# ebiggers/libdeflate

Hardware: AMD Instinct MI355X
Metric: compress+decompress MB/s, 64 KiB chunks level 6 (higher is better)
Workload: dtype u8

## Files before the change

### libdeflate_amd/csrc/checksum_kernels.hip

```cpp
#include "device_common.h"
#include "kernels.h"

#define CRC_POLY 0xEDB88320u
#define ROW 1024u

static __device__ __forceinline__ u32 gf2_mulmod(u32 a, u32 b)
{
	u32 p = 0;
#pragma unroll 8
	for (int i = 31; i >= 0; i--) {
		p ^= b & (0u - ((a >> i) & 1u));
		b = (b >> 1) ^ (CRC_POLY & (0u - (b & 1u)));
	}
	return p;
}

struct crc_lds {
	u32 stride[16][256];
	u32 t0[256];
};

static __device__ __forceinline__ u32
crc_row_generic(const crc_lds &L, const u32 *__restrict__ xpow8,
		const u8 *__restrict__ p, u32 len, u32 reg, u32 lane)
{
	u32 start = lane * 16;
	u32 r = (lane == 0) ? reg : 0;
	u32 part = 0;

	if (start < len) {
		u32 m = len - start;
		if (m > 16)
			m = 16;
		for (u32 k = 0; k < m; k++)
			r = L.t0[(r ^ p[start + k]) & 0xFF] ^ (r >> 8);
		part = gf2_mulmod(xpow8[len - start - m], r);
	} else if (lane == 0) {
		part = r;
	}
	return wave_xor(part);
}

static __device__ __forceinline__ u32
crc_row_full_final(const crc_lds &L, const u32 *__restrict__ xpow8,
		   uint4 v, u32 reg_lane, u32 lane)
{
	u32 w[4] = { v.x ^ reg_lane, v.y, v.z, v.w };
	u32 r = 0;
#pragma unroll
	for (int i = 0; i < 4; i++) {
#pragma unroll
		for (int j = 0; j < 4; j++)
			r = L.t0[(r ^ (w[i] >> (8 * j))) & 0xFF] ^ (r >> 8);
	}
	return wave_xor(gf2_mulmod(xpow8[(63 - lane) * 16], r));
}

extern "C" __global__ void __launch_bounds__(256)
lda_crc32_batch_kernel(u64 n_chunks, const u8 *__restrict__ base,
		       const u64 *__restrict__ offsets,
		       const u64 *__restrict__ nbytes,
		       const u32 *__restrict__ init,
		       u32 *__restrict__ out,
		       const u32 *__restrict__ g_tables ,
		       const u32 *__restrict__ xpow8 )
{
	__shared__ crc_lds L;
	const u32 lane = threadIdx.x & 63;
	const u32 wave = threadIdx.x >> 6;

	for (u32 i = threadIdx.x; i < 17 * 256; i += 256)
		((u32 *)&L)[i] = g_tables[i];
	__syncthreads();

	for (u64 c = (u64)blockIdx.x * 4 + wave; c < n_chunks;
	     c += (u64)gridDim.x * 4) {
		const u8 *p = base + offsets[c];
		u64 n = nbytes[c];
		u32 reg = ~(init ? init[c] : 0u);

		u32 head = (u32)((0 - (uintptr_t)p) & 15);
		if (head > n)
			head = (u32)n;
		if (head) {
			reg = crc_row_generic(L, xpow8, p, head, reg, lane);
			p += head;
			n -= head;
		}
		u64 rows = n / ROW;
		if (rows) {
			const uint4 *q = (const uint4 *)p + lane;
			u32 r = (lane == 0) ? reg : 0;
			uint4 v = q[0];
			for (u64 row = 0; row + 1 < rows; row++) {
				uint4 nv = q[(row + 1) * 64];
				u32 w0 = v.x ^ r, w1 = v.y, w2 = v.z, w3 = v.w;
				r = L.stride[0][w0 & 0xFF] ^
				    L.stride[1][(w0 >> 8) & 0xFF] ^
				    L.stride[2][(w0 >> 16) & 0xFF] ^
				    L.stride[3][w0 >> 24] ^
				    L.stride[4][w1 & 0xFF] ^
				    L.stride[5][(w1 >> 8) & 0xFF] ^
				    L.stride[6][(w1 >> 16) & 0xFF] ^
				    L.stride[7][w1 >> 24] ^
				    L.stride[8][w2 & 0xFF] ^
				    L.stride[9][(w2 >> 8) & 0xFF] ^
				    L.stride[10][(w2 >> 16) & 0xFF] ^
				    L.stride[11][w2 >> 24] ^
				    L.stride[12][w3 & 0xFF] ^
				    L.stride[13][(w3 >> 8) & 0xFF] ^
				    L.stride[14][(w3 >> 16) & 0xFF] ^
				    L.stride[15][w3 >> 24];
				v = nv;
			}
			reg = crc_row_full_final(L, xpow8, v, r, lane);
			p += rows * ROW;
			n -= rows * ROW;
		}
		if (n)
			reg = crc_row_generic(L, xpow8, p, (u32)n, reg, lane);
		if (lane == 0)
			out[c] = ~reg;
	}
}


#define ADLER_MOD 65521u
#define ADLER_SEG (1u << 24)

static __device__ __forceinline__ u32 dot4(u32 bytes, u32 weights, u32 acc)
{
	return __builtin_amdgcn_udot4(bytes, weights, acc, false);
}

extern "C" __global__ void __launch_bounds__(256)
lda_adler32_batch_kernel(u64 n_chunks, const u8 *__restrict__ base,
			 const u64 *__restrict__ offsets,
			 const u64 *__restrict__ nbytes,
			 const u32 *__restrict__ init,
			 u32 *__restrict__ out)
{
	const u32 lane = threadIdx.x & 63;
	const u32 wave = threadIdx.x >> 6;

	for (u64 c = (u64)blockIdx.x * 4 + wave; c < n_chunks;
	     c += (u64)gridDim.x * 4) {
		const u8 *p = base + offsets[c];
		u64 left = nbytes[c];
		u32 a0 = init ? init[c] : 1u;
		u64 s1 = a0 & 0xFFFF, s2 = a0 >> 16;

		while (left) {
			u32 n = left > ADLER_SEG ? ADLER_SEG : (u32)left;
			u64 S = 0, W = 0;
			u32 pos = 0;
			u32 head = (u32)((0 - (uintptr_t)p) & 15);

			if (head > n)
				head = n;
			if (lane < head) {
				u32 b = p[lane];
				S += b;
				W += (u64)(n - lane) * b;
			}
			pos = head;
			u32 rows = (n - pos) / ROW;
			const uint4 *q = (const uint4 *)(p + pos) + lane;
			for (u32 row = 0; row < rows; row++) {
				uint4 v = q[(u64)row * 64];
				u32 o = pos + row * ROW + lane * 16;
				u32 bs = dot4(v.x, 0x01010101u, 0);
				bs = dot4(v.y, 0x01010101u, bs);
				bs = dot4(v.z, 0x01010101u, bs);
				bs = dot4(v.w, 0x01010101u, bs);
				u32 ks = dot4(v.x, 0x03020100u, 0);
				ks = dot4(v.y, 0x07060504u, ks);
				ks = dot4(v.z, 0x0B0A0908u, ks);
				ks = dot4(v.w, 0x0F0E0D0Cu, ks);
				S += bs;
				W += (u64)(n - o) * bs - ks;
			}
			pos += rows * ROW;
			for (u32 i = pos + lane; i < n; i += 64) {
				u32 b = p[i];
				S += b;
				W += (u64)(n - i) * b;
			}
			S = wave_sum64(S);
			W = wave_sum64(W);
			s2 = (s2 + (u64)n % ADLER_MOD * s1 + W % ADLER_MOD) % ADLER_MOD;
			s1 = (s1 + S) % ADLER_MOD;
			p += n;
			left -= n;
		}
		if (lane == 0)
			out[c] = (u32)((s2 << 16) | s1);
	}
}

extern "C" __global__ void
lda_dict_prep_kernel(const u8 *__restrict__ dict, u64 dict_nbytes, u32 tail,
		     u32 pre_len, u32 sinfo, u8 *__restrict__ blk)
{
	if (threadIdx.x == 0) {
		((u32 *)blk)[0] = sinfo;
		((u64 *)blk)[2] = 0;
		((u64 *)blk)[3] = dict_nbytes;
	}
	const u32 skip = pre_len - tail;
	const u8 *src = dict + dict_nbytes - tail;
	for (u32 i = threadIdx.x; i < pre_len; i += blockDim.x)
		blk[64 + i] = i < skip ? 0 : src[i - skip];
}
```

### libdeflate_amd/csrc/host_common.h

```cpp
#ifndef LDA_HOST_COMMON_H
#define LDA_HOST_COMMON_H

#include <hip/hip_runtime.h>
#include <stddef.h>
#include <stdint.h>
#include <atomic>
#include <exception>
#include <functional>
#include <mutex>

#include "../../include/libdeflate_amd.h"

namespace lda {

void set_error(const char *fmt, ...);

#define LDA_HIP_TRY(expr, failret)                                           \
	do {                                                                 \
		hipError_t e_ = (expr);                                      \
		if (e_ != hipSuccess) {                                      \
			lda::set_error("%s: %s", #expr, hipGetErrorString(e_)); \
			return failret;                                      \
		}                                                            \
	} while (0)
// ... 5 lines not shown
	} while (0)
#define LDA_TRY(expr) LDA_HIP_TRY(expr, false)

struct DeviceCtx {
	int device = -1;
	int num_cus = 0;
	uint32_t *d_crc_tables = nullptr;
	uint32_t *d_crc_xpow8 = nullptr;
	std::mutex stage_mu;
	void *d_stage = nullptr;
	size_t stage_cap = 0;
	std::atomic<bool> deflate_attr_set{false}, inflate_attr_set{false}, stream_attr_set{false};
	std::atomic<int> sizes_waves_fit{0};
};

DeviceCtx *device_ctx();
bool device_selfcheck(int num_cus, uint64_t out[5]);

struct DeviceGuard {
	int prev = -1;
	bool switched = false, good = true;
	explicit DeviceGuard(int device);
	~DeviceGuard();
	bool ok() const { return good; }
	DeviceGuard(const DeviceGuard &) = delete;
	DeviceGuard &operator=(const DeviceGuard &) = delete;
};

struct EnvCfg {
	bool no_small = false;
	bool no_segments = false;
	int inflate_lpw = 0;
	bool inflate_par = true;
	int inflate_waves_per_cu = 16;
	int sizes_waves_per_cu = 0;
	int host_threads = 4;
	size_t seg_bytes = 0;
	bool no_stream_par = false;
	size_t stream_par_min = 16384;
	size_t zip_large_min = (size_t)128 << 10;
	size_t stream_window = 0;
	size_t stream_chunk = 0;
	int devices = 1;
	bool no_selfcheck = false;
	bool bgzf_serial = false;
	bool tar_serial = false;
	bool fanout_oversub = false;
	bool compress_overlap = true;
	int compress_tail_rounds = 0;
};
const EnvCfg &env_cfg();

void *stage_reserve(DeviceCtx *ctx, size_t nbytes);

[[noreturn]] void die(const char *what);

void complain(const char *what, int status);

struct PinnedPair {
	uint8_t *buf[2] = { nullptr, nullptr };
	hipEvent_t ev[2] = { nullptr, nullptr };
	size_t cap = 0;
	bool ensure(size_t want);
	void release();
};
struct PinnedBuf {
// ... 92 lines not shown
```

### libdeflate_amd/csrc/host_context.hip

```cpp
#include <stdarg.h>
#include <stdio.h>
#include <stdlib.h>
#include <string.h>
#include <pthread.h>
#include <algorithm>
#include <condition_variable>
#include <deque>
#include <functional>
#include <memory>
#include <thread>
#include <vector>

#include "host_common.h"
#include "kernels.h"

namespace lda {

static thread_local char g_err[512] = "";

void set_error(const char *fmt, ...)
{
	va_list ap;
	va_start(ap, fmt);
	vsnprintf(g_err, sizeof(g_err), fmt, ap);
	va_end(ap);
}

[[noreturn]] void die(const char *what)
{
	fprintf(stderr,
		"libdeflate_amd: %s failed on the gfx950 device (%s) and this "
		"call has no error return. This library has no CPU fallback.\n",
		what, g_err);
	abort();
}

void complain(const char *what, int status)
{
	fprintf(stderr, "libdeflate_amd: %s: status %d (%s)\n", what, status, g_err);
}

static EnvCfg read_env()
{
	EnvCfg c;
	c.no_small = getenv("LDA_NO_SMALL") != nullptr;
	c.no_segments = getenv("LDA_NO_SEGMENTS") != nullptr;
	if (const char *e = getenv("LDA_INFLATE_LPW")) {
		int v = atoi(e);
		if (v >= 1 && v <= 64)
			c.inflate_lpw = v;
	}
	if (const char *e = getenv("LDA_INFLATE_PAR"))
		c.inflate_par = atoi(e) != 0;
	if (const char *e = getenv("LDA_HOST_THREADS")) {
		int v = atoi(e);
		if (v >= 1 && v <= 16)
			c.host_threads = v;
	}
	if (const char *e = getenv("LDA_INFLATE_WAVES_PER_CU")) {
		int v = atoi(e);
		if (v >= 1 && v <= 16)
			c.inflate_waves_per_cu = v;
	}
	if (const char *e = getenv("LDA_SIZES_WAVES_PER_CU")) {
		int v = atoi(e);
		if (v >= 1 && v <= 32)
			c.sizes_waves_per_cu = v;
	}
	if (const char *e = getenv("LDA_SEG_BYTES")) {
		size_t v = (size_t)strtoull(e, nullptr, 0);
		if (v >= 8192 && v <= 65536 && v % 4096 == 0)
			c.seg_bytes = v;
	}
	c.no_stream_par = getenv("LDA_NO_STREAM_PAR") != nullptr;
	if (const char *e = getenv("LDA_STREAM_PAR_MIN"))
		c.stream_par_min = (size_t)strtoull(e, nullptr, 0);
	if (const char *e = getenv("LDA_ZIP_LARGE_MIN")) {
		size_t v = (size_t)strtoull(e, nullptr, 0);
		if (v >= 1)
			c.zip_large_min = v;
	}
	if (const char *e = getenv("LDA_STREAM_WINDOW")) {
		c.stream_window = (size_t)strtoull(e, nullptr, 0);
		if (c.stream_window && c.stream_window < 32768)
			c.stream_window = 32768;
	}
// ... 554 lines not shown

int span_out(PinnedPair *pp, const uint8_t *d_base, uint64_t d_off, uint8_t *dst, size_t n,
	     hipStream_t st, size_t piece)
{
	const size_t P = piece ? piece : span_piece(n), np = (n + P - 1) / P;
	std::vector<void *> outs(np);
	std::vector<uint64_t> nb(np), off(np);
	for (size_t i = 0; i < np; i++) {
		outs[i] = dst + i * P;
		nb[i] = i + 1 < np ? P : n - i * P;
		off[i] = d_off + i * P;
	}
	return copy_out_packed(pp, d_base, np, outs.data(), nb.data(), off.data(), st);
}

#define MAX_DEVICES 16
static DeviceCtx g_ctx[MAX_DEVICES];
static std::mutex g_ctx_mu;

static void gen_crc_tables(uint32_t *tab , uint32_t *xpow )
{
	const uint32_t poly = 0xEDB88320u;
	uint32_t t0[256];

	for (uint32_t b = 0; b < 256; b++) {
		uint32_t r = b;
		for (int k = 0; k < 8; k++)
			r = (r >> 1) ^ (poly & (0u - (r & 1u)));
		t0[b] = r;
	}
	for (uint32_t b = 0; b < 256; b++) {
		uint32_t r = t0[b];
		int zeros = 0;
		for (int k = 15; k >= 0; k--) {
			int want = (15 - k) + 1008;
			for (; zeros < want; zeros++)
				r = t0[r & 0xFF] ^ (r >> 8);
			tab[k * 256 + b] = r;
		}
	}
	memcpy(tab + 16 * 256, t0, sizeof(t0));
	uint32_t x = 0x80000000u;
	for (int d = 0; d < 1024; d++) {
		xpow[d] = x;
		for (int k = 0; k < 8; k++)
			x = (x >> 1) ^ (poly & (0u - (x & 1u)));
	}
}

bool device_selfcheck(int num_cus, uint64_t out[5])
{
	const unsigned blocks = (unsigned)(num_cus > 0 ? num_cus : 256);
	const unsigned waves = 16 * blocks;
	const size_t region = lda_selfcheck_region_bytes();
	uint8_t *buf = nullptr;
	uint64_t *d_cnt = nullptr;

	memset(out, 0, 5 * sizeof(uint64_t));
	LDA_HIP_TRY(hipMalloc((void **)&buf, (size_t)waves * region + 64), false);
	d_cnt = (uint64_t *)(buf + (size_t)waves * region);
	hipError_t e = hipMemset(buf, 0, (size_t)waves * region + 64);
	if (e == hipSuccess) {
		hipLaunchKernelGGL(lda_selfcheck_lds_order_kernel, dim3(blocks), dim3(1024), 0, 0,
				   d_cnt);
		hipLaunchKernelGGL(lda_selfcheck_visibility_kernel, dim3(waves), dim3(64), 0, 0,
				   buf, d_cnt);
		e = hipGetLastError();
	}
	if (e == hipSuccess)
		e = hipMemcpy(out, d_cnt, 5 * sizeof(uint64_t), hipMemcpyDeviceToHost);
	(void)hipFree(buf);
	if (e != hipSuccess) {
		set_error("hardware self-check: %s", hipGetErrorString(e));
		return false;
// ... 22 lines not shown
		good = false;
		return;
	}
	switched = true;
}

DeviceGuard::~DeviceGuard()
{
	if (switched && prev >= 0)
		(void)hipSetDevice(prev);
}

DeviceCtx *device_ctx()
{
	int dev = -1;
	hipError_t e = hipGetDevice(&dev);

	if (e != hipSuccess || dev < 0 || dev >= MAX_DEVICES) {
		set_error("hipGetDevice: %s", hipGetErrorString(e));
		return nullptr;
	}
	std::lock_guard<std::mutex> lk(g_ctx_mu);
	DeviceCtx *c = &g_ctx[dev];
	if (c->device == dev)
		return c;

	hipDeviceProp_t prop;
	LDA_HIP_TRY(hipGetDeviceProperties(&prop, dev), nullptr);
	if (strncmp(prop.gcnArchName, "gfx950", 6) != 0) {
		set_error("device %d is %s, this build targets gfx950 only",
			  dev, prop.gcnArchName);
		return nullptr;
	}
	static uint32_t tab[LDA_CRC_TABLE_WORDS], xpow[LDA_CRC_XPOW_WORDS];
	gen_crc_tables(tab, xpow);
	uint32_t *d_tab = nullptr;
	LDA_HIP_TRY(hipMalloc((void **)&d_tab, sizeof(tab) + sizeof(xpow)), nullptr);
	hipError_t ce = hipMemcpy(d_tab, tab, sizeof(tab), hipMemcpyHostToDevice);
	if (ce == hipSuccess)
		ce = hipMemcpy(d_tab + LDA_CRC_TABLE_WORDS, xpow, sizeof(xpow),
			       hipMemcpyHostToDevice);
	if (ce != hipSuccess) {
		(void)hipFree(d_tab);
		set_error("hipMemcpy(CRC tables): %s", hipGetErrorString(ce));
		return nullptr;
	}
	if (!env_cfg().no_selfcheck) {
		uint64_t sc[5];
		if (!device_selfcheck(prop.multiProcessorCount, sc)) {
			(void)hipFree(d_tab);
			return nullptr;
		}
	}
	c->d_crc_tables = d_tab;
	c->d_crc_xpow8 = d_tab + LDA_CRC_TABLE_WORDS;
	c->num_cus = prop.multiProcessorCount;
	c->device = dev;
	return c;
}

void *stage_reserve(DeviceCtx *ctx, size_t nbytes)
{
	if (nbytes <= ctx->stage_cap)
		return ctx->d_stage;
	size_t cap = align_up(nbytes + nbytes / 4 + 4096, 4096);
	void *p = nullptr;
	if (ctx->d_stage)
		(void)hipFree(ctx->d_stage);
	ctx->d_stage = nullptr;
	ctx->stage_cap = 0;
	hipError_t e = hipMalloc(&p, cap);
	if (e != hipSuccess) {
		set_error("hipMalloc(%zu): %s", cap, hipGetErrorString(e));
		return nullptr;
// ... 34 lines not shown
```

### libdeflate_amd/csrc/host_decompress.hip

```cpp
#include <stdio.h>
#include <stdlib.h>
#include <atomic>
#include <new>
#include <string.h>
#include <vector>

#include "host_objects.h"
#include "kernels.h"

namespace lda {

malloc_func_t g_malloc = nullptr;
free_func_t g_free = nullptr;

void *DevBuf::reserve(size_t n)
{
	if (n <= cap)
		return p;
	release();
	size_t want = align_up(n + n / 8 + 4096, 4096);
	hipError_t e = hipMalloc(&p, want);
	if (e != hipSuccess) {
		p = nullptr;
		set_error("hipMalloc(%zu): %s", want, hipGetErrorString(e));
// ... 171 lines not shown
	if (dict) {
		dlen = (uint32_t)(dict_nbytes < 32768 ? dict_nbytes : 32768);
		dtail = (const uint8_t *)d_dict + dict_nbytes - dlen;
		uint8_t *blk = s + blk_at;
		hipLaunchKernelGGL(lda_dict_prep_kernel, dim3(1), dim3(64), 0, st,
				   (const uint8_t *)d_dict, (uint64_t)dict_nbytes, 0u, 0u, 0u, blk);
		LDA_HIP_TRY(hipGetLastError(), LIBDEFLATE_AMD_NO_DEVICE);
		if (format == LIBDEFLATE_AMD_ZLIB) {
			dict_id = (uint32_t *)(blk + 4);
			int rc = libdeflate_amd_adler32_batch(1, d_dict, (const uint64_t *)(blk + 16),
							      (const uint64_t *)(blk + 24), NULL, dict_id,
							      stream);
			if (rc != LIBDEFLATE_AMD_OK)
				return rc;
		}
	}
	uint32_t *sums = (uint32_t *)s;
	uint64_t *ain = d_actual_in ? d_actual_in : (uint64_t *)(s + sums_bytes);
	uint64_t *aout = d_actual_out ? d_actual_out :
			 (uint64_t *)(s + sums_bytes + 8 * n);
	int exact_fill = d_actual_out == NULL;

	uint32_t lpw_max = 64;
	while (lda_inflate_lds_per_stream() * lpw_max + lda_inflate_lds_shared() > 163840)
		lpw_max >>= 1;
	uint32_t lpw = 2;
	while (lpw < lpw_max && (size_t)lpw * 32 * (size_t)c->num_cus < n)
		lpw <<= 1;
	if (env_cfg().inflate_lpw)
		lpw = (uint32_t)env_cfg().inflate_lpw;
	if (lpw > lpw_max)
		lpw = lpw_max;
	const bool par = env_cfg().inflate_par;
	if (!c->inflate_attr_set.load(std::memory_order_acquire)) {
		LDA_HIP_TRY(hipFuncSetAttribute(
				(const void *)lda_inflate_batch_kernel,
				hipFuncAttributeMaxDynamicSharedMemorySize,
				(int)(lda_inflate_lds_per_stream() * lpw_max +
				      lda_inflate_lds_shared())),
			    LIBDEFLATE_AMD_NO_DEVICE);
		c->inflate_attr_set.store(true, std::memory_order_release);
	}
	if (par) {
		const size_t grid_max = (size_t)c->num_cus * inflate_waves_per_cu();
		size_t grid = grid_max < n ? grid_max : n;
		const size_t tok_bytes = grid * lda_inflate_tokcap() * 4;
		uint32_t *tok = (uint32_t *)d->tokens.reserve(inflate_tokens_bytes(n, c->num_cus));
		if (!tok)
			return LIBDEFLATE_AMD_OOM;
		uint32_t *next = (uint32_t *)((uint8_t *)tok + tok_bytes);
		LDA_HIP_TRY(hipMemsetAsync(next, 0, 16, st), LIBDEFLATE_AMD_NO_DEVICE);
		uint32_t *order = NULL;
		if (n > grid && n < 0xFFFFFFFFull) {
			order = (uint32_t *)(s + sums_bytes + 16 * n);
			hipLaunchKernelGGL(lda_inflate_order_kernel, dim3(1), dim3(1024), 0, st,
					   (uint64_t)n, d_in_nbytes, d_out_avail, order);
		}
		size_t lds = inflate_wave_lds();
		hipLaunchKernelGGL(lda_inflate_wave_kernel, dim3((unsigned)grid),
				   dim3(64), lds, st, (uint64_t)n, format, tok, next,
				   (const uint32_t *)order,
				   (const uint8_t *)d_in, d_in_offsets, d_in_nbytes,
				   (uint8_t *)d_out, d_out_offsets, d_out_avail,
				   d_results, ain, aout, dtail, dlen, (const uint32_t *)dict_id);
	} else {
		size_t lds = lda_inflate_lds_per_stream() * lpw +
			     lda_inflate_lds_shared();
		hipLaunchKernelGGL(lda_inflate_batch_kernel,
				   dim3((unsigned)((n + lpw - 1) / lpw)), dim3(64),
				   lds, st, (uint64_t)n, format, lpw,
				   (const uint8_t *)d_in, d_in_offsets, d_in_nbytes,
				   (uint8_t *)d_out, d_out_offsets, d_out_avail,
				   d_results, ain, aout, dtail, dlen, (const uint32_t *)dict_id);
	}
	LDA_HIP_TRY(hipGetLastError(), LIBDEFLATE_AMD_NO_DEVICE);
	if (format != LIBDEFLATE_AMD_DEFLATE) {
		int rc = format == LIBDEFLATE_AMD_GZIP ?
			libdeflate_amd_crc32_batch(n, d_out, d_out_offsets, aout,
						   NULL, sums, stream) :
			libdeflate_amd_adler32_batch(n, d_out, d_out_offsets,
						     aout, NULL, sums, stream);
		if (rc != LIBDEFLATE_AMD_OK)
			return rc;
	}
	if (format != LIBDEFLATE_AMD_DEFLATE || exact_fill) {
		hipLaunchKernelGGL(lda_inflate_finalize_kernel,
				   dim3((unsigned)((n + 255) / 256)), dim3(256), 0,
				   st, (uint64_t)n, format, exact_fill,
				   (const uint8_t *)d_in, d_in_offsets, d_out_avail,
				   sums, d_results, ain, aout);
		LDA_HIP_TRY(hipGetLastError(), LIBDEFLATE_AMD_NO_DEVICE);
	}
	return LIBDEFLATE_AMD_OK;
}

extern "C" LIBDEFLATEAPI int
libdeflate_amd_decompress_batch(struct libdeflate_decompressor *d, int format,
				size_t n, const void *d_in,
				const uint64_t *d_in_offsets,
				const uint64_t *d_in_nbytes, void *d_out,
				const uint64_t *d_out_offsets,
				const uint64_t *d_out_avail, int32_t *d_results,
				uint64_t *d_actual_in, uint64_t *d_actual_out,
				void *stream)
{
	return decompress_batch_impl(d, format, n, d_in, d_in_offsets, d_in_nbytes, d_out,
				     d_out_offsets, d_out_avail, d_results, d_actual_in,
				     d_actual_out, stream);
// ... 420 lines not shown
```

### libdeflate_amd/csrc/inflate_kernel.hip

```cpp
#include "device_common.h"
#include "kernels.h"

#ifndef PAR_PRIO
#define PAR_PRIO 1
#endif
#ifndef LIT_TB
#define LIT_TB 10
#endif
#ifndef LIT_TB_MIN
#define LIT_TB_MIN 9
#endif
#ifndef OFF_TB
#define OFF_TB 8
#endif
#ifndef OFF_TB_MIN
#define OFF_TB_MIN 7
#endif
#define TB_BIG_BLOCK 8192u

#define K_LIT (0u << 14)
#define K_LEN (1u << 14)
#define K_EOB (2u << 14)
#define ENTRY(kind, payload, len) ((u16)((kind) | ((payload) << 4) | (len)))

// ... 2100 lines not shown
			u64 ain = (CONSUMED() + 7) / 8;
			if (ain > in_n)
				result = LDA_BAD_DATA;
			else if (!COUNT || actual_in)
				actual_in[c] = hdr + ain;
		}
		if (COUNT) {
			if (result == LDA_SUCCESS && format == LDA_FMT_GZIP) {
				const u8 *p = inp + (CONSUMED() + 7) / 8;
				const u32 isize = p[4] | ((u32)p[5] << 8) | ((u32)p[6] << 16) |
						  ((u32)p[7] << 24);
				if (isize != (u32)out_pos)
					result = LDA_BAD_DATA;
			}
			if (result == LDA_SUCCESS && actual_in && format != LDA_FMT_DEFLATE)
				actual_in[c] += format == LDA_FMT_GZIP ? 8 : 4;
			if (result != LDA_SUCCESS && actual_in)
				actual_in[c] = 0;
			results[c] = result;
			actual_out[c] = result == LDA_SUCCESS ? out_pos : 0;
			return;
		}
		results[c] = result;
		actual_out[c] = result == LDA_SUCCESS ? out_pos :
				PREFIX && result == LDA_PREFIX ? out_avail : 0;
		if (result != LDA_SUCCESS)
			actual_in[c] = 0;
	}
}
#undef ltb
#undef otb

#ifndef LDA_INFLATE_DEVICE_ONLY
extern "C" __global__ void __launch_bounds__(64, 4)
lda_inflate_batch_kernel(u64 n_chunks, int format, u32 lpw,
			 const u8 *__restrict__ in_base,
			 const u64 *__restrict__ in_offsets,
			 const u64 *__restrict__ in_nbytes,
			 u8 *__restrict__ out_base,
			 const u64 *__restrict__ out_offsets,
			 const u64 *__restrict__ out_avail_arr,
			 s32 *__restrict__ results,
			 u64 *__restrict__ actual_in,
			 u64 *__restrict__ actual_out,
			 const u8 *__restrict__ dict, u32 dict_len,
			 const u32 *__restrict__ dict_id)
{
	lu8 *lds_raw = (lu8 *)(uintptr_t)0;

	inflate_block(blockIdx.x, lds_raw, 0, NULL, n_chunks, format, lpw, in_base,
		      in_offsets, in_nbytes, out_base, out_offsets, out_avail_arr,
		      results, actual_in, actual_out, dict, dict_len, dict_id);
}

#ifndef PAR_WAVES_PER_SIMD
#define PAR_WAVES_PER_SIMD 4
#endif
static __device__ __forceinline__ u32
order_bucket(const u64 *__restrict__ in_nbytes, const u64 *__restrict__ out_avail, u64 i)
{
	u64 b = in_nbytes[i];
	if (out_avail && b + (b >> 5) >= out_avail[i])
		b >>= 4;
	b >>= 9;
	return 255 - (b < 255 ? (u32)b : 255u);
}

extern "C" __global__ void __launch_bounds__(1024)
lda_inflate_order_kernel(u64 n, const u64 *__restrict__ in_nbytes,
			 const u64 *__restrict__ out_avail,
			 u32 *__restrict__ order)
{
	__shared__ u32 cnt[256], at[256];
	const u32 tid = threadIdx.x;

	if (tid < 256)
		cnt[tid] = 0;
	__syncthreads();
	for (u64 i = tid; i < n; i += 1024)
		atomicAdd(&cnt[order_bucket(in_nbytes, out_avail, i)], 1u);
	__syncthreads();
	if (tid < 64) {
		u32 v[4], s = 0;
#pragma unroll
		for (u32 k = 0; k < 4; k++) {
			v[k] = cnt[4 * tid + k];
			s += v[k];
		}
		u32 base = wave_scan_incl(s) - s;
#pragma unroll
		for (u32 k = 0; k < 4; k++) {
			at[4 * tid + k] = base;
			base += v[k];
		}
	}
	__syncthreads();
	for (u64 i = tid; i < n; i += 1024)
		order[atomicAdd(&at[order_bucket(in_nbytes, out_avail, i)], 1u)] = (u32)i;
}

extern "C" __global__ void __launch_bounds__(64, PAR_WAVES_PER_SIMD)
lda_inflate_wave_kernel(u64 n_chunks, int format, u32 *__restrict__ tokscratch,
			u32 *__restrict__ next_stream,
			const u32 *__restrict__ order,
			const u8 *__restrict__ in_base,
			const u64 *__restrict__ in_offsets,
			const u64 *__restrict__ in_nbytes,
			u8 *__restrict__ out_base,
			const u64 *__restrict__ out_offsets,
			const u64 *__restrict__ out_avail_arr,
			s32 *__restrict__ results,
			u64 *__restrict__ actual_in,
			u64 *__restrict__ actual_out,
			const u8 *__restrict__ dict, u32 dict_len,
			const u32 *__restrict__ dict_id)
{
	lu8 *lds_raw = (lu8 *)(uintptr_t)0;
	u32 *tok = tokscratch + (size_t)blockIdx.x * PAR_SCRATCH;

	u32 first = blockIdx.x;
	if (gridDim.x > 1) {
		const u32 m = (2u << (31 - __builtin_clz(gridDim.x - 1))) - 1;
		do
			first = (first ^ (first >> 3) ^ (first >> 6) ^ (first >> 9)) & m;
		while (first >= gridDim.x);
	}
	for (u64 blk = first; blk < n_chunks;) {
		inflate_block(order ? order[blk] : blk, lds_raw, 1, tok, n_chunks, format, 1, in_base,
			      in_offsets, in_nbytes, out_base, out_offsets,
			      out_avail_arr, results, actual_in, actual_out, dict, dict_len,
			      dict_id);
		wave_sync();
		u32 nx = 0;
		if (lane_id() == 0)
			nx = atomicAdd(next_stream, 1u);
		blk = (u64)gridDim.x + bcast_first(nx);
	}
}

extern "C" size_t lda_inflate_tokcap(void)
{
	return PAR_SCRATCH;
}

extern "C" size_t lda_inflate_window_bytes(void)
{
	return PAR_RW + PAR_STAGE_BYTES + PAR_MAP_BYTES;
}

extern "C" size_t lda_inflate_lds_per_stream(void)
{
	return sizeof(struct stream_lds);
}

extern "C" size_t lda_inflate_lds_shared(void)
{
	return sizeof(struct shared_lds);
}

extern "C" __global__ void
lda_inflate_finalize_kernel(u64 n_chunks, int format, int exact_fill,
			    const u8 *__restrict__ in_base,
			    const u64 *__restrict__ in_offsets,
			    const u64 *__restrict__ out_avail,
// ... 43 lines not shown
```

### libdeflate_amd/csrc/kernels.h

```cpp
#ifndef LDA_KERNELS_H
#define LDA_KERNELS_H

#include <hip/hip_runtime.h>
#include <stdint.h>

#include "large_plan.h"

extern "C" __global__ void
lda_crc32_batch_kernel(uint64_t n_chunks, const uint8_t *base,
		       const uint64_t *offsets, const uint64_t *nbytes,
		       const uint32_t *init, uint32_t *out,
		       const uint32_t *g_tables, const uint32_t *xpow8);
extern "C" __global__ void
lda_adler32_batch_kernel(uint64_t n_chunks, const uint8_t *base,
			 const uint64_t *offsets, const uint64_t *nbytes,
			 const uint32_t *init, uint32_t *out);
#define LDA_DICT_BLK_HDR 64
extern "C" __global__ void
lda_dict_prep_kernel(const uint8_t *dict, uint64_t dict_nbytes, uint32_t tail,
		     uint32_t pre_len, uint32_t sinfo, uint8_t *blk);

extern "C" __global__ void
lda_inflate_batch_kernel(uint64_t n_chunks, int format, uint32_t lpw,
			 const uint8_t *in_base,
			 const uint64_t *in_offsets, const uint64_t *in_nbytes,
			 uint8_t *out_base, const uint64_t *out_offsets,
			 const uint64_t *out_avail, int32_t *results,
			 uint64_t *actual_in, uint64_t *actual_out,
			 const uint8_t *dict, uint32_t dict_len,
			 const uint32_t *dict_id);
extern "C" __global__ void
lda_inflate_wave_kernel(uint64_t n_chunks, int format, uint32_t *tokscratch,
			uint32_t *next_stream, const uint32_t *order,
			const uint8_t *in_base,
			const uint64_t *in_offsets, const uint64_t *in_nbytes,
			uint8_t *out_base, const uint64_t *out_offsets,
			const uint64_t *out_avail, int32_t *results,
			uint64_t *actual_in, uint64_t *actual_out,
			const uint8_t *dict, uint32_t dict_len,
			const uint32_t *dict_id);
extern "C" __global__ void
lda_inflate_order_kernel(uint64_t n, const uint64_t *in_nbytes, const uint64_t *out_avail,
			 uint32_t *order);
extern "C" __global__ void
lda_inflate_sizes_kernel(uint64_t n_chunks, int format, uint32_t par, uint32_t *next_stream,
			 const uint32_t *order, const uint8_t *in_base,
			 const uint64_t *in_offsets, const uint64_t *in_nbytes,
			 const uint64_t *limits, int32_t *results, uint64_t *actual_in,
			 uint64_t *out_nbytes, uint32_t dict_len, const uint32_t *dict_id);
extern "C" size_t lda_inflate_sizes_lds_bytes(void);
extern "C" __global__ void
lda_packed_round_kernel(uint64_t n, uint64_t align_mask, const uint64_t *sizes,
			uint64_t *rounded);
extern "C" __global__ void
lda_packed_desc_kernel(uint64_t n, uint64_t capacity, const uint64_t *in_nbytes,
		       const uint64_t *sizes, const uint64_t *block_sums, uint64_t *offsets,
		       int32_t *verdict, uint64_t *dec_in_nbytes, uint64_t *dec_avail);
extern "C" __global__ void
lda_packed_merge_kernel(uint64_t n, const int32_t *verdict, int32_t *results,
			uint64_t *actual_in, uint64_t *actual_out);
extern "C" __global__ void
lda_inflate_prefix_kernel(uint64_t n_chunks, int format, uint32_t par, uint32_t *tokscratch,
			  uint32_t *next_stream, const uint32_t *order, const uint8_t *in_base,
			  const uint64_t *in_offsets, const uint64_t *in_nbytes,
			  uint8_t *out_base, const uint64_t *out_offsets, const uint64_t *limits,
			  int32_t *results, uint64_t *actual_in, uint64_t *actual_out,
			  const uint8_t *dict, uint32_t dict_len, const uint32_t *dict_id);
extern "C" __global__ void
lda_gzm_peek_desc_kernel(uint64_t max_members, uint64_t n, uint64_t head, const uint64_t *result,
			 const uint64_t *index, uint64_t *in_off, uint64_t *in_n, uint64_t *out_off,
			 uint64_t *limits, int32_t *results, uint64_t *head_nbytes);
extern "C" size_t lda_inflate_tokcap(void);
extern "C" size_t lda_inflate_window_bytes(void);
// ... 442 lines not shown
#define LDA_SHUF_VERD_OWN ((uint64_t)1 << 63)
extern "C" __global__ void
lda_unshuffle_kernel(uint64_t n_u, uint64_t n_tiles, const uint64_t *u_tile_end,
		     const uint64_t *u_src, const uint64_t *u_dst, const uint64_t *u_geom,
		     const uint8_t *ws, const uint8_t *alt, uint8_t *out);
extern "C" __global__ void
lda_shuf_final_kernel(uint64_t n, const uint64_t *verd, const int32_t *decode, int32_t *results);
extern "C" __global__ void
lda_shuffle_kernel(uint64_t n_u, uint64_t n_tiles, const uint64_t *u_tile_end,
		   const uint64_t *u_src, const uint64_t *u_dst, const uint64_t *u_geom,
		   const uint8_t *in, uint8_t *rooms);
extern "C" __global__ void
lda_shufw_chunk_kernel(uint64_t n, int format, const uint64_t *first, const uint64_t *count,
		       const uint64_t *usize, const uint64_t *pc_off, const uint64_t *pc_n,
		       const uint64_t *out_n, const uint32_t *sums, uint64_t *csize, uint32_t *sum,
		       uint64_t *sizes);
extern "C" __global__ void
lda_shufw_place_kernel(uint64_t n, int format, int level, uint64_t out_avail,
		       const uint64_t *ecols, const uint64_t *pc_off, const uint64_t *pc_n,
		       const uint64_t *slot_off, const uint64_t *out_n, const uint64_t *csize,
		       const uint32_t *sum, const uint64_t *offsets, const uint64_t *block_sums,
		       uint8_t *out, uint64_t *cp_src, uint64_t *cp_dst, uint64_t *cp_len,
		       uint64_t *index);
extern "C" __global__ void
lda_shufw_final_kernel(uint64_t n, uint64_t raw_total, uint64_t out_avail,
		       const uint64_t *total_at, uint64_t *result);

extern "C" __global__ void
lda_selfcheck_lds_order_kernel(uint64_t *counters);
extern "C" __global__ void
lda_selfcheck_visibility_kernel(uint8_t *buf, uint64_t *counters);
extern "C" size_t lda_selfcheck_region_bytes(void);

#define LDA_CRC_TABLE_WORDS (17 * 256)
#define LDA_CRC_XPOW_WORDS 1024

#endif
```

Measured before the change: 34980.

## Fuse checksum verification into inflate wave kernel and halve CRC stride tables

Each stream's gzip CRC32 or zlib Adler-32 is now computed and checked at the end of the wave-parallel inflate kernel, reusing that wave's LDS for the CRC tables. This replaces the separate checksum batch kernel launch and its second read of the output. The CRC row step now uses two independent 8-table chains instead of one 16-table chain, with a 4-row load-ahead, which halves the LDS tables. Risks are added latency per stream inside the inflate kernel and extra register pressure that may lower occupancy of the inflate kernel.

```diff
diff --git a/libdeflate_amd/csrc/checksum_device.h b/libdeflate_amd/csrc/checksum_device.h
--- /dev/null
+++ b/libdeflate_amd/csrc/checksum_device.h
@@ -0,0 +1,224 @@
+#ifndef LDA_CHECKSUM_DEVICE_H
+#define LDA_CHECKSUM_DEVICE_H
+
+#include "device_common.h"
+
+#define CRC_POLY 0xEDB88320u
+#define CRC_ROW 1024u
+#define CRC_STRIDE_WORDS (8u * 256u)
+#define CRC_LDS_WORDS (9u * 256u)
+#define CRC_AHEAD 4u
+
+static __device__ __forceinline__ u32 gf2_mulmod(u32 a, u32 b)
+{
+	u32 p = 0;
+#pragma unroll 8
+	for (int i = 31; i >= 0; i--) {
+		p ^= b & (0u - ((a >> i) & 1u));
+		b = (b >> 1) ^ (CRC_POLY & (0u - (b & 1u)));
+	}
+	return p;
+}
+
+template <class TP> static __device__ __forceinline__ void
+crc_tables_load(TP T, const u32 *__restrict__ g_tables, bool stride, u32 lane)
+{
+	const uint4 *g = (const uint4 *)g_tables;
+	uint4 v[CRC_LDS_WORDS / 256];
+
+#pragma unroll
+	for (u32 k = 0; k < CRC_LDS_WORDS / 256; k++)
+		if (stride || k == CRC_STRIDE_WORDS / 256)
+			v[k] = g[64 * k + lane];
+#pragma unroll
+	for (u32 k = 0; k < CRC_LDS_WORDS / 256; k++)
+		if (stride || k == CRC_STRIDE_WORDS / 256) {
+			const u32 i = 4 * (64 * k + lane);
+			T[i] = v[k].x;
+			T[i + 1] = v[k].y;
+			T[i + 2] = v[k].z;
+			T[i + 3] = v[k].w;
+		}
+}
+
+template <class TP> static __device__ __forceinline__ u32
+crc_row_generic(TP t0, const u32 *__restrict__ xpow8,
+		const u8 *__restrict__ p, u32 len, u32 reg, u32 lane)
+{
+	u32 start = lane * 16;
+	u32 r = (lane == 0) ? reg : 0;
+	u32 part = 0;
+
+	if (start < len) {
+		u32 m = len - start;
+		if (m > 16)
+			m = 16;
+		u32 w[4] = { 0, 0, 0, 0 };
+		if (m == 16) {
+			__builtin_memcpy(w, p + start, 16);
+		} else {
+#pragma unroll
+			for (u32 k = 0; k < 15; k++) {
+				const u32 b = p[start + (k < m ? k : m - 1)];
+				w[k >> 2] |= (k < m ? b : 0u) << (8 * (k & 3));
+			}
+		}
+#pragma unroll
+		for (u32 k = 0; k < 16; k++)
+			if (k < m)
+				r = t0[(r ^ (w[k >> 2] >> (8 * (k & 3)))) & 0xFF] ^ (r >> 8);
+		part = gf2_mulmod(xpow8[len - start - m], r);
+	} else if (lane == 0) {
+		part = r;
+	}
+	return wave_xor(part);
+}
+
+template <class TP> static __device__ __forceinline__ u32
+crc_row_full_final(TP t0, const u32 *__restrict__ xpow8, uint4 v, u32 r0, u32 r1, u32 lane)
+{
+	u32 w[4] = { v.x ^ r0, v.y, v.z ^ r1, v.w };
+	u32 r = 0;
+#pragma unroll
+	for (int i = 0; i < 4; i++) {
+#pragma unroll
+		for (int j = 0; j < 4; j++)
+			r = t0[(r ^ (w[i] >> (8 * j))) & 0xFF] ^ (r >> 8);
+	}
+	return wave_xor(gf2_mulmod(xpow8[(63 - lane) * 16], r));
+}
+
+template <class TP> static __device__ __forceinline__ u32
+crc_row_step(TP S, u32 r, u32 lo, u32 hi)
+{
+	const u32 w0 = lo ^ r, w1 = hi;
+
+	return S[0 * 256 + (w0 & 0xFF)] ^
+	       S[1 * 256 + ((w0 >> 8) & 0xFF)] ^
+	       S[2 * 256 + ((w0 >> 16) & 0xFF)] ^
+	       S[3 * 256 + (w0 >> 24)] ^
+	       S[4 * 256 + (w1 & 0xFF)] ^
+	       S[5 * 256 + ((w1 >> 8) & 0xFF)] ^
+	       S[6 * 256 + ((w1 >> 16) & 0xFF)] ^
+	       S[7 * 256 + (w1 >> 24)];
+}
+
+template <class TP> static __device__ __forceinline__ u32
+crc32_wave(TP T, const u32 *__restrict__ xpow8, const u8 *__restrict__ p, u64 n,
+	   u32 reg, u32 lane)
+{
+	TP t0 = T + CRC_STRIDE_WORDS;
+
+	u32 head = (u32)((0 - (uintptr_t)p) & 15);
+	if (head > n)
+		head = (u32)n;
+	if (head) {
+		reg = crc_row_generic(t0, xpow8, p, head, reg, lane);
+		p += head;
+		n -= head;
+	}
+	u64 rows = n / CRC_ROW;
+	if (rows) {
+		const uint4 *q = (const uint4 *)p + lane;
+		u32 r0 = (lane == 0) ? reg : 0, r1 = 0;
+		const u64 last = rows - 1;
+		const uint4 vlast = q[last * 64];
+		uint4 v[CRC_AHEAD];
+#pragma unroll
+		for (u32 k = 0; k < CRC_AHEAD; k++)
+			v[k] = q[(k < last ? k : last) * 64];
+		u64 row = 0;
+		for (; row + CRC_AHEAD <= last; row += CRC_AHEAD) {
+#pragma unroll
+			for (u32 k = 0; k < CRC_AHEAD; k++) {
+				const uint4 cur = v[k];
+				const u64 nx = row + k + CRC_AHEAD;
+				v[k] = q[(nx < last ? nx : last) * 64];
+				r0 = crc_row_step(T, r0, cur.x, cur.y);
+				r1 = crc_row_step(T, r1, cur.z, cur.w);
+			}
+		}
+#pragma unroll
+		for (u32 k = 0; k + 1 < CRC_AHEAD; k++)
+			if (row + k < last) {
+				r0 = crc_row_step(T, r0, v[k].x, v[k].y);
+				r1 = crc_row_step(T, r1, v[k].z, v[k].w);
+			}
+		reg = crc_row_full_final(t0, xpow8, vlast, r0, r1, lane);
+		p += rows * CRC_ROW;
+		n -= rows * CRC_ROW;
+	}
+	if (n)
+		reg = crc_row_generic(t0, xpow8, p, (u32)n, reg, lane);
+	return reg;
+}
+
+static __device__ __forceinline__ bool crc32_wave_needs_stride(const u8 *p, u64 n)
+{
+	const u64 head = (0 - (uintptr_t)p) & 15;
+
+	return n >= head + 2 * CRC_ROW;
+}
+
+
+#define ADLER_MOD 65521u
+#define ADLER_SEG (1u << 24)
+
+static __device__ __forceinline__ u32 dot4(u32 bytes, u32 weights, u32 acc)
+{
+	return __builtin_amdgcn_udot4(bytes, weights, acc, false);
+}
+
+static __device__ __forceinline__ u32
+adler32_wave(const u8 *__restrict__ p, u64 left, u32 a0, u32 lane)
+{
+	u64 s1 = a0 & 0xFFFF, s2 = a0 >> 16;
+
+	while (left) {
+		u32 n = left > ADLER_SEG ? ADLER_SEG : (u32)left;
+		u64 S = 0, W = 0;
+		u32 pos = 0;
+		u32 head = (u32)((0 - (uintptr_t)p) & 15);
+
+		if (head > n)
+			head = n;
+		if (lane < head) {
+			u32 b = p[lane];
+			S += b;
+			W += (u64)(n - lane) * b;
+		}
+		pos = head;
+		u32 rows = (n - pos) / CRC_ROW;
+		const uint4 *q = (const uint4 *)(p + pos) + lane;
+#pragma unroll 4
+		for (u32 row = 0; row < rows; row++) {
+			uint4 v = q[(u64)row * 64];
+			u32 o = pos + row * CRC_ROW + lane * 16;
+			u32 bs = dot4(v.x, 0x01010101u, 0);
+			bs = dot4(v.y, 0x01010101u, bs);
+			bs = dot4(v.z, 0x01010101u, bs);
+			bs = dot4(v.w, 0x01010101u, bs);
+			u32 ks = dot4(v.x, 0x03020100u, 0);
+			ks = dot4(v.y, 0x07060504u, ks);
+			ks = dot4(v.z, 0x0B0A0908u, ks);
+			ks = dot4(v.w, 0x0F0E0D0Cu, ks);
+			S += bs;
+			W += (u64)(n - o) * bs - ks;
+		}
+		pos += rows * CRC_ROW;
+		for (u32 i = pos + lane; i < n; i += 64) {
+			u32 b = p[i];
+			S += b;
+			W += (u64)(n - i) * b;
+		}
+		S = wave_sum64(S);
+		W = wave_sum64(W);
+		s2 = (s2 + (u64)n % ADLER_MOD * s1 + W % ADLER_MOD) % ADLER_MOD;
+		s1 = (s1 + S) % ADLER_MOD;
+		p += n;
+		left -= n;
+	}
+	return (u32)((s2 << 16) | s1);
+}
+
+#endif
diff --git a/libdeflate_amd/csrc/checksum_kernels.hip b/libdeflate_amd/csrc/checksum_kernels.hip
--- a/libdeflate_amd/csrc/checksum_kernels.hip
+++ b/libdeflate_amd/csrc/checksum_kernels.hip
@@ -1,60 +1,6 @@
 #include "device_common.h"
 #include "kernels.h"
-
-#define CRC_POLY 0xEDB88320u
-#define ROW 1024u
-
-static __device__ __forceinline__ u32 gf2_mulmod(u32 a, u32 b)
-{
-	u32 p = 0;
-#pragma unroll 8
-	for (int i = 31; i >= 0; i--) {
-		p ^= b & (0u - ((a >> i) & 1u));
-		b = (b >> 1) ^ (CRC_POLY & (0u - (b & 1u)));
-	}
-	return p;
-}
-
-struct crc_lds {
-	u32 stride[16][256];
-	u32 t0[256];
-};
-
-static __device__ __forceinline__ u32
-crc_row_generic(const crc_lds &L, const u32 *__restrict__ xpow8,
-		const u8 *__restrict__ p, u32 len, u32 reg, u32 lane)
-{
-	u32 start = lane * 16;
-	u32 r = (lane == 0) ? reg : 0;
-	u32 part = 0;
-
-	if (start < len) {
-		u32 m = len - start;
-		if (m > 16)
-			m = 16;
-		for (u32 k = 0; k < m; k++)
-			r = L.t0[(r ^ p[start + k]) & 0xFF] ^ (r >> 8);
-		part = gf2_mulmod(xpow8[len - start - m], r);
-	} else if (lane == 0) {
-		part = r;
-	}
-	return wave_xor(part);
-}
-
-static __device__ __forceinline__ u32
-crc_row_full_final(const crc_lds &L, const u32 *__restrict__ xpow8,
-		   uint4 v, u32 reg_lane, u32 lane)
-{
-	u32 w[4] = { v.x ^ reg_lane, v.y, v.z, v.w };
-	u32 r = 0;
-#pragma unroll
-	for (int i = 0; i < 4; i++) {
-#pragma unroll
-		for (int j = 0; j < 4; j++)
-			r = L.t0[(r ^ (w[i] >> (8 * j))) & 0xFF] ^ (r >> 8);
-	}
-	return wave_xor(gf2_mulmod(xpow8[(63 - lane) * 16], r));
-}
+#include "checksum_device.h"
 
 extern "C" __global__ void __launch_bounds__(256)
 lda_crc32_batch_kernel(u64 n_chunks, const u8 *__restrict__ base,
@@ -65,72 +11,21 @@
 		       const u32 *__restrict__ g_tables ,
 		       const u32 *__restrict__ xpow8 )
 {
-	__shared__ crc_lds L;
+	__shared__ __attribute__((aligned(16))) u32 T[CRC_LDS_WORDS];
 	const u32 lane = threadIdx.x & 63;
 	const u32 wave = threadIdx.x >> 6;
 
-	for (u32 i = threadIdx.x; i < 17 * 256; i += 256)
-		((u32 *)&L)[i] = g_tables[i];
+	for (u32 i = threadIdx.x; i < CRC_LDS_WORDS; i += 256)
+		T[i] = g_tables[i];
 	__syncthreads();
 
 	for (u64 c = (u64)blockIdx.x * 4 + wave; c < n_chunks;
 	     c += (u64)gridDim.x * 4) {
-		const u8 *p = base + offsets[c];
-		u64 n = nbytes[c];
-		u32 reg = ~(init ? init[c] : 0u);
-
-		u32 head = (u32)((0 - (uintptr_t)p) & 15);
-		if (head > n)
-			head = (u32)n;
-		if (head) {
-			reg = crc_row_generic(L, xpow8, p, head, reg, lane);
-			p += head;
-			n -= head;
-		}
-		u64 rows = n / ROW;
-		if (rows) {
-			const uint4 *q = (const uint4 *)p + lane;
-			u32 r = (lane == 0) ? reg : 0;
-			uint4 v = q[0];
-			for (u64 row = 0; row + 1 < rows; row++) {
-				uint4 nv = q[(row + 1) * 64];
-				u32 w0 = v.x ^ r, w1 = v.y, w2 = v.z, w3 = v.w;
-				r = L.stride[0][w0 & 0xFF] ^
-				    L.stride[1][(w0 >> 8) & 0xFF] ^
-				    L.stride[2][(w0 >> 16) & 0xFF] ^
-				    L.stride[3][w0 >> 24] ^
-				    L.stride[4][w1 & 0xFF] ^
-				    L.stride[5][(w1 >> 8) & 0xFF] ^
-				    L.stride[6][(w1 >> 16) & 0xFF] ^
-				    L.stride[7][w1 >> 24] ^
-				    L.stride[8][w2 & 0xFF] ^
-				    L.stride[9][(w2 >> 8) & 0xFF] ^
-				    L.stride[10][(w2 >> 16) & 0xFF] ^
-				    L.stride[11][w2 >> 24] ^
-				    L.stride[12][w3 & 0xFF] ^
-				    L.stride[13][(w3 >> 8) & 0xFF] ^
-				    L.stride[14][(w3 >> 16) & 0xFF] ^
-				    L.stride[15][w3 >> 24];
-				v = nv;
-			}
-			reg = crc_row_full_final(L, xpow8, v, r, lane);
-			p += rows * ROW;
-			n -= rows * ROW;
-		}
-		if (n)
-			reg = crc_row_generic(L, xpow8, p, (u32)n, reg, lane);
+		const u32 reg = crc32_wave((const u32 *)T, xpow8, base + offsets[c], nbytes[c],
+					   ~(init ? init[c] : 0u), lane);
 		if (lane == 0)
 			out[c] = ~reg;
 	}
-}
-
-
-#define ADLER_MOD 65521u
-#define ADLER_SEG (1u << 24)
-
-static __device__ __forceinline__ u32 dot4(u32 bytes, u32 weights, u32 acc)
-{
-	return __builtin_amdgcn_udot4(bytes, weights, acc, false);
 }
 
 extern "C" __global__ void __launch_bounds__(256)
@@ -145,56 +40,9 @@
 
 	for (u64 c = (u64)blockIdx.x * 4 + wave; c < n_chunks;
 	     c += (u64)gridDim.x * 4) {
-		const u8 *p = base + offsets[c];
-		u64 left = nbytes[c];
-		u32 a0 = init ? init[c] : 1u;
-		u64 s1 = a0 & 0xFFFF, s2 = a0 >> 16;
-
-		while (left) {
-			u32 n = left > ADLER_SEG ? ADLER_SEG : (u32)left;
-			u64 S = 0, W = 0;
-			u32 pos = 0;
-			u32 head = (u32)((0 - (uintptr_t)p) & 15);
-
-			if (head > n)
-				head = n;
-			if (lane < head) {
-				u32 b = p[lane];
-				S += b;
-				W += (u64)(n - lane) * b;
-			}
-			pos = head;
-			u32 rows = (n - pos) / ROW;
-			const uint4 *q = (const uint4 *)(p + pos) + lane;
-			for (u32 row = 0; row < rows; row++) {
-				uint4 v = q[(u64)row * 64];
-				u32 o = pos + row * ROW + lane * 16;
-				u32 bs = dot4(v.x, 0x01010101u, 0);
-				bs = dot4(v.y, 0x01010101u, bs);
-				bs = dot4(v.z, 0x01010101u, bs);
-				bs = dot4(v.w, 0x01010101u, bs);
-				u32 ks = dot4(v.x, 0x03020100u, 0);
-				ks = dot4(v.y, 0x07060504u, ks);
-				ks = dot4(v.z, 0x0B0A0908u, ks);
-				ks = dot4(v.w, 0x0F0E0D0Cu, ks);
-				S += bs;
-				W += (u64)(n - o) * bs - ks;
-			}
-			pos += rows * ROW;
-			for (u32 i = pos + lane; i < n; i += 64) {
-				u32 b = p[i];
-				S += b;
-				W += (u64)(n - i) * b;
-			}
-			S = wave_sum64(S);
-			W = wave_sum64(W);
-			s2 = (s2 + (u64)n % ADLER_MOD * s1 + W % ADLER_MOD) % ADLER_MOD;
-			s1 = (s1 + S) % ADLER_MOD;
-			p += n;
-			left -= n;
-		}
+		const u32 a = adler32_wave(base + offsets[c], nbytes[c], init ? init[c] : 1u, lane);
 		if (lane == 0)
-			out[c] = (u32)((s2 << 16) | s1);
+			out[c] = a;
 	}
 }
 
diff --git a/libdeflate_amd/csrc/host_common.h b/libdeflate_amd/csrc/host_common.h
--- a/libdeflate_amd/csrc/host_common.h
+++ b/libdeflate_amd/csrc/host_common.h
@@ -61,6 +61,7 @@
 	bool no_segments = false;
 	int inflate_lpw = 0;
 	bool inflate_par = true;
+	bool inflate_fused_check = true;
 	int inflate_waves_per_cu = 16;
 	int sizes_waves_per_cu = 0;
 	int host_threads = 4;
diff --git a/libdeflate_amd/csrc/host_context.hip b/libdeflate_amd/csrc/host_context.hip
--- a/libdeflate_amd/csrc/host_context.hip
+++ b/libdeflate_amd/csrc/host_context.hip
@@ -52,6 +52,8 @@
 	}
 	if (const char *e = getenv("LDA_INFLATE_PAR"))
 		c.inflate_par = atoi(e) != 0;
+	if (const char *e = getenv("LDA_INFLATE_FUSED_CHECK"))
+		c.inflate_fused_check = atoi(e) != 0;
 	if (const char *e = getenv("LDA_HOST_THREADS")) {
 		int v = atoi(e);
 		if (v >= 1 && v <= 16)
@@ -672,14 +674,14 @@
 	for (uint32_t b = 0; b < 256; b++) {
 		uint32_t r = t0[b];
 		int zeros = 0;
-		for (int k = 15; k >= 0; k--) {
-			int want = (15 - k) + 1008;
+		for (int k = 7; k >= 0; k--) {
+			int want = (7 - k) + 1016;
 			for (; zeros < want; zeros++)
 				r = t0[r & 0xFF] ^ (r >> 8);
 			tab[k * 256 + b] = r;
 		}
 	}
-	memcpy(tab + 16 * 256, t0, sizeof(t0));
+	memcpy(tab + 8 * 256, t0, sizeof(t0));
 	uint32_t x = 0x80000000u;
 	for (int d = 0; d < 1024; d++) {
 		xpow[d] = x;
@@ -768,14 +770,13 @@
 			  dev, prop.gcnArchName);
 		return nullptr;
 	}
-	static uint32_t tab[LDA_CRC_TABLE_WORDS], xpow[LDA_CRC_XPOW_WORDS];
-	gen_crc_tables(tab, xpow);
+	static uint32_t tab[LDA_CRC_TABLE_WORDS + LDA_CRC_XPOW_WORDS];
+	gen_crc_tables(tab, tab + LDA_CRC_TABLE_WORDS);
 	uint32_t *d_tab = nullptr;
-	LDA_HIP_TRY(hipMalloc((void **)&d_tab, sizeof(tab) + sizeof(xpow)), nullptr);
+	LDA_HIP_TRY(hipMalloc((void **)&d_tab, sizeof(tab)), nullptr);
 	hipError_t ce = hipMemcpy(d_tab, tab, sizeof(tab), hipMemcpyHostToDevice);
 	if (ce == hipSuccess)
-		ce = hipMemcpy(d_tab + LDA_CRC_TABLE_WORDS, xpow, sizeof(xpow),
-			       hipMemcpyHostToDevice);
+		ce = lda_inflate_set_crc_tables(tab);
 	if (ce != hipSuccess) {
 		(void)hipFree(d_tab);
 		set_error("hipMemcpy(CRC tables): %s", hipGetErrorString(ce));
diff --git a/libdeflate_amd/csrc/host_decompress.hip b/libdeflate_amd/csrc/host_decompress.hip
--- a/libdeflate_amd/csrc/host_decompress.hip
+++ b/libdeflate_amd/csrc/host_decompress.hip
@@ -227,6 +227,7 @@
 	if (lpw > lpw_max)
 		lpw = lpw_max;
 	const bool par = env_cfg().inflate_par;
+	const bool fused = par && env_cfg().inflate_fused_check;
 	if (!c->inflate_attr_set.load(std::memory_order_acquire)) {
 		LDA_HIP_TRY(hipFuncSetAttribute(
 				(const void *)lda_inflate_batch_kernel,
@@ -257,7 +258,11 @@
 				   (const uint32_t *)order,
 				   (const uint8_t *)d_in, d_in_offsets, d_in_nbytes,
 				   (uint8_t *)d_out, d_out_offsets, d_out_avail,
-				   d_results, ain, aout, dtail, dlen, (const uint32_t *)dict_id);
+				   d_results, ain, aout, dtail, dlen, (const uint32_t *)dict_id,
+				   fused && (format != LIBDEFLATE_AMD_DEFLATE || exact_fill) ?
+					   (uint64_t)(uintptr_t)sums | LDA_FINISH_FUSED |
+						   (exact_fill ? LDA_FINISH_EXACT_FILL : 0) :
+					   (uint64_t)0);
 	} else {
 		size_t lds = lda_inflate_lds_per_stream() * lpw +
 			     lda_inflate_lds_shared();
@@ -269,6 +274,8 @@
 				   d_results, ain, aout, dtail, dlen, (const uint32_t *)dict_id);
 	}
 	LDA_HIP_TRY(hipGetLastError(), LIBDEFLATE_AMD_NO_DEVICE);
+	if (fused)
+		return LIBDEFLATE_AMD_OK;
 	if (format != LIBDEFLATE_AMD_DEFLATE) {
 		int rc = format == LIBDEFLATE_AMD_GZIP ?
 			libdeflate_amd_crc32_batch(n, d_out, d_out_offsets, aout,
diff --git a/libdeflate_amd/csrc/inflate_kernel.hip b/libdeflate_amd/csrc/inflate_kernel.hip
--- a/libdeflate_amd/csrc/inflate_kernel.hip
+++ b/libdeflate_amd/csrc/inflate_kernel.hip
@@ -2156,6 +2156,8 @@
 #undef otb
 
 #ifndef LDA_INFLATE_DEVICE_ONLY
+#include "checksum_device.h"
+
 extern "C" __global__ void __launch_bounds__(64, 4)
 lda_inflate_batch_kernel(u64 n_chunks, int format, u32 lpw,
 			 const u8 *__restrict__ in_base,
@@ -2221,6 +2223,77 @@
 	__syncthreads();
 	for (u64 i = tid; i < n; i += 1024)
 		order[atomicAdd(&at[order_bucket(in_nbytes, out_avail, i)], 1u)] = (u32)i;
+}
+
+static_assert(CRC_LDS_WORDS == LDA_CRC_TABLE_WORDS, "the device table is loaded as it lies");
+static_assert(CRC_LDS_WORDS * 4 <= sizeof(struct stream_lds) + sizeof(struct shared_lds) +
+				   PAR_RW + PAR_STAGE_BYTES + PAR_MAP_BYTES,
+	      "the CRC tables must fit the LDS the wave already owns");
+static __device__ __attribute__((aligned(16))) u32
+	lda_inflate_crc_tab[LDA_CRC_TABLE_WORDS + LDA_CRC_XPOW_WORDS];
+
+extern "C" hipError_t lda_inflate_set_crc_tables(const u32 *tables_xpow8)
+{
+	return hipMemcpyToSymbol(HIP_SYMBOL(lda_inflate_crc_tab), tables_xpow8,
+				 sizeof(lda_inflate_crc_tab), 0, hipMemcpyHostToDevice);
+}
+
+static __device__ __forceinline__ void
+finish_stream(u64 c, lu8 *lds_raw, int format, int finish,
+	      const u8 *__restrict__ in_base, const u64 *__restrict__ in_offsets,
+	      const u8 *out_base, const u64 *__restrict__ out_offsets,
+	      const u64 *__restrict__ out_avail, s32 *results, u64 *actual_in,
+	      u64 *actual_out, u32 *__restrict__ sums)
+{
+	const u32 *crc_tables = lda_inflate_crc_tab;
+	u32 lane = threadIdx.x;
+	asm volatile("" : "+v"(lane), "+s"(format), "+s"(finish));
+
+	global_stores_visible();
+	const s32 r = (s32)bcast_first((u32)results[c]);
+	const u64 n = bcast64(actual_out[c]);
+	const bool fill_ok = !(finish & LDA_FINISH_EXACT_FILL) || n == out_avail[c];
+
+	if (format == LDA_FMT_DEFLATE) {
+		if (lane == 0 && r == LDA_SUCCESS && !fill_ok)
+			results[c] = LDA_SHORT_OUTPUT;
+		return;
+	}
+	const u8 *p = out_base + out_offsets[c];
+	u32 sum = 0;
+	if (format == LDA_FMT_ZLIB) {
+		sum = adler32_wave(p, n, 1u, lane);
+	} else if (n) {
+		lu32 *T = (lu32 *)lds_raw;
+		crc_tables_load(T, crc_tables, crc32_wave_needs_stride(p, n), lane);
+		wave_sync();
+		sum = ~crc32_wave((const lu32 *)T, crc_tables + CRC_LDS_WORDS, p, n, ~0u, lane);
+	}
+	if (lane != 0)
+		return;
+	sums[c] = sum;
+	if (r != LDA_SUCCESS)
+		return;
+	if (!fill_ok) {
+		results[c] = LDA_SHORT_OUTPUT;
+		return;
+	}
+	const u64 ain = actual_in[c];
+	const u8 *f = in_base + in_offsets[c] + ain;
+	if (format == LDA_FMT_ZLIB) {
+		const u32 want = ((u32)f[0] << 24) | ((u32)f[1] << 16) | ((u32)f[2] << 8) | f[3];
+		if (want != sum)
+			results[c] = LDA_BAD_DATA;
+		else
+			actual_in[c] = ain + 4;
+	} else {
+		const u32 want = f[0] | ((u32)f[1] << 8) | ((u32)f[2] << 16) | ((u32)f[3] << 24);
+		const u32 isize = f[4] | ((u32)f[5] << 8) | ((u32)f[6] << 16) | ((u32)f[7] << 24);
+		if (want != sum || isize != (u32)n)
+			results[c] = LDA_BAD_DATA;
+		else
+			actual_in[c] = ain + 8;
+	}
 }
 
 extern "C" __global__ void __launch_bounds__(64, PAR_WAVES_PER_SIMD)
@@ -2237,7 +2310,8 @@
 			u64 *__restrict__ actual_in,
 			u64 *__restrict__ actual_out,
 			const u8 *__restrict__ dict, u32 dict_len,
-			const u32 *__restrict__ dict_id)
+			const u32 *__restrict__ dict_id,
+			u64 finish_sums)
 {
 	lu8 *lds_raw = (lu8 *)(uintptr_t)0;
 	u32 *tok = tokscratch + (size_t)blockIdx.x * PAR_SCRATCH;
@@ -2254,6 +2328,13 @@
 			      in_offsets, in_nbytes, out_base, out_offsets,
 			      out_avail_arr, results, actual_in, actual_out, dict, dict_len,
 			      dict_id);
+		u64 bf = blk, fs = finish_sums;
+		asm volatile("" : "+s"(bf), "+s"(fs));
+		if (fs) {
+			finish_stream(order ? order[bf] : bf, lds_raw, format, (int)(fs & 15), in_base,
+				      in_offsets, out_base, out_offsets, out_avail_arr, results,
+				      actual_in, actual_out, (u32 *)(uintptr_t)(fs & ~(u64)15));
+		}
 		wave_sync();
 		u32 nx = 0;
 		if (lane_id() == 0)
diff --git a/libdeflate_amd/csrc/kernels.h b/libdeflate_amd/csrc/kernels.h
--- a/libdeflate_amd/csrc/kernels.h
+++ b/libdeflate_amd/csrc/kernels.h
@@ -38,7 +38,11 @@
 			const uint64_t *out_avail, int32_t *results,
 			uint64_t *actual_in, uint64_t *actual_out,
 			const uint8_t *dict, uint32_t dict_len,
-			const uint32_t *dict_id);
+			const uint32_t *dict_id,
+			uint64_t finish_sums);
+#define LDA_FINISH_FUSED 1
+#define LDA_FINISH_EXACT_FILL 2
+extern "C" hipError_t lda_inflate_set_crc_tables(const uint32_t *tables_xpow8);
 extern "C" __global__ void
 lda_inflate_order_kernel(uint64_t n, const uint64_t *in_nbytes, const uint64_t *out_avail,
 			 uint32_t *order);
@@ -547,7 +551,7 @@
 lda_selfcheck_visibility_kernel(uint8_t *buf, uint64_t *counters);
 extern "C" size_t lda_selfcheck_region_bytes(void);
 
-#define LDA_CRC_TABLE_WORDS (17 * 256)
+#define LDA_CRC_TABLE_WORDS (9 * 256)
 #define LDA_CRC_XPOW_WORDS 1024
 
 #endif
```

After: 35200, median of 6. Within noise of the previous version (+0.6%).
